# scienstanford/pbrt-v3-spectral

Measured on AMD Instinct MI355X. Metric: Mray/s (killeroo-simple, PathIntegrator maxdepth 5, Halton, SampledSpectrum-31, 1024 spp), higher is better.
Workload: dtype f32

## Files before the change

pbrt-v3-spectral_amd/csrc/device/pt_kernels.hip:

```cpp
#include <hip/hip_runtime.h>
#include <algorithm>
#include <chrono>
#include <cmath>
#include <cstdio>
#include <cstdlib>
#include <thread>
#include <cstring>
#include <string>
#include <vector>
#include <type_traits>
#include "d_sampling.h"
#include "d_texture.h"
#include "d_lens.h"

using namespace dpt;

#ifdef MIPT_PART
#define MIPT_HAS_MAIN (MIPT_PART == 0)
#else
#define MIPT_HAS_MAIN 1
#endif

namespace dptk {

// ... 8 lines not shown
        if (e_ != hipSuccess) {                                                           \
            g_err = std::string(#x) + ": " + hipGetErrorString(e_);                       \
            return MI_ERR_HIP;                                                            \
        }                                                                                 \
    } while (0)

constexpr int BLOCK = 256;
#ifndef MIPT_STACK_LDS
#define MIPT_STACK_LDS 12
#endif
constexpr int STACK_LDS = MIPT_STACK_LDS;
constexpr int STACK_SPILL = 64 - STACK_LDS;
static_assert(STACK_LDS >= 1 && STACK_LDS <= 63 && STACK_LDS * BLOCK * 12 <= 160 * 1024, "MIPT_STACK_LDS: 1..63 entries, and the block's stack must fit the CU's LDS");

enum : int {
    P_FILMX = 0, P_FILMY,
    P_TENC0, P_TENC1, P_TENC2, P_TENC3,
    P_COUNT
};
constexpr int P_WEIGHT = P_COUNT;
constexpr int P_LENSDIFF = P_COUNT + 1, N_LENSDIFF = 12;
enum : int {
    R_RAY0 = 0,
    R_RAY1,
    R_SH0, R_SH1,
    R_MI0, R_MI1,
    R_HIT,
    R_COUNT
};
constexpr int NQ = 8;
enum : int {
    Q_L = 0,
    Q_BETA = NQ,
    Q_LB = 2 * NQ,
    Q_LMIS = 3 * NQ,
    Q_COUNT = 4 * NQ,
    Q_LCA = Q_COUNT
};
DEV float Get4(const float4 &v, int k) { return k == 0 ? v.x : (k == 1 ? v.y : (k == 2 ? v.z : v.w)); }
DEV void Set4(float4 &v, int k, float x) { if (k == 0) v.x = x; else if (k == 1) v.y = x; else if (k == 2) v.z = x; else v.w = x; }
enum : int { I_HITPRIM = 0, I_PIXEL, I_SAMPLE, I_IDXLO, I_IDXHI, I_DIM , I_FLAGS, I_MISLIGHT,
             I_NPEND, I_PEND0, I_PEND1, I_PEND2, I_PEND3,
             I_BAND,
             I_HITINST,
             I_COUNT };
constexpr int MAX_PEND = 4;
constexpr int PEND_OVERFLOW = 0x100;
enum : int {
    F_ALIVE = 1, F_FINISHED = 2, F_SPECULAR = 4, F_SHADOW = 8, F_MIS = 16, F_NEE = 32, F_A_ADDED = 64,
    F_L_IN_B = 128,
    F_L_ZERO = 256,
    F_BETA_ONE = 512,
    F_DIFF = 1024,
    F_CAND = 2048, F_NEE_NZ = 4096,
    F_MIS_DARK = 8192
};
constexpr int FLAG_BITS = 14, FLAG_MASK = (1 << FLAG_BITS) - 1, BOUNCE_SHIFT = 14, DIM_SHIFT = 22;
static_assert(F_MIS_DARK < (1 << FLAG_BITS), "slot flags outgrew their field");
DEV int LPlane(int flags) { return (flags & F_L_IN_B) ? Q_LB : Q_L; }
DEV int LOtherPlane(int flags) { return (flags & F_L_IN_B) ? Q_L : Q_LB; }
DEV int StateWord(int flags, int bounces, int dim) { return (flags & FLAG_MASK) | ((bounces & 0xff) << BOUNCE_SHIFT) | (int)((unsigned)(dim & 0x3ff) << DIM_SHIFT); }
DEV int StateBounces(int word) { return (word >> BOUNCE_SHIFT) & 0xff; }
DEV int StateDim(int word) { return (int)((unsigned)word >> DIM_SHIFT); }
DEV bool RaySpanInBox(const V3 &o, const V3 &d, const float4 &bmin, const float4 &bmax, float *spanLo, float *spanHi) {
    float t0 = 0.f, t1 = kInfinity;
    const float oo[3] = {o.x, o.y, o.z}, dd[3] = {d.x, d.y, d.z}, lo[3] = {bmin.x, bmin.y, bmin.z}, hi[3] = {bmax.x, bmax.y, bmax.z};
#pragma unroll
    for (int a = 0; a < 3; ++a) {
        if (dd[a] == 0.f) { if (oo[a] < lo[a] || oo[a] > hi[a]) return false; continue; }
        const float inv = 1.f / dd[a];
        float ta = (lo[a] - oo[a]) * inv, tb = (hi[a] - oo[a]) * inv;
        if (ta > tb) { const float tt = ta; ta = tb; tb = tt; }
        tb *= 1.0001f;
        if (ta > t0) t0 = ta;
        if (tb < t1) t1 = tb;
    }
    *spanLo = t0; *spanHi = t1;
    return !(t0 > t1);
}
constexpr unsigned MIS_EXCL_BITS = 27, MIS_EXCL_NONE = (1u << MIS_EXCL_BITS) - 1u;
DEV void MisSpanWords(float lo, float hi, unsigned prim, float *tHi, float *word) {
    const float w = 1.f - lo / hi;
    int c = 126 - (int)((__float_as_uint(w) >> 23) & 0xffu);
    if (!(w > 0.f)) c = 20;
    c = (lo > 0.f && hi < kInfinity) ? max(0, min(c, 20)) : 0;
    *tHi = hi;
    *word = __uint_as_float(prim | ((unsigned)c << MIS_EXCL_BITS));
}

constexpr int MAX_CLASSES = 16;
constexpr int MISS_CLASS = 15;

struct Pool {
    float *f;
    float4 *q;
    float4 *r;
    int *i;
    uint32_t *shadowQ, *misQ;
    uint32_t *extQ;
    uint32_t *shadeQ;
    uint32_t *ovfQ;
    uint32_t n;
    __host__ __device__ __forceinline__ size_t ScalarIndex(int plane, uint32_t slot) const { return (size_t)plane * n + slot; }
    __host__ __device__ __forceinline__ size_t QuadIndex(int plane, uint32_t slot) const { return (((size_t)(plane >> 3) * n + slot) << 3) + (plane & 7); }
    __host__ __device__ __forceinline__ size_t RecordIndex(int plane, uint32_t slot) const {
        return plane < R_HIT ? (((size_t)(plane >> 1) * n + slot) << 1) + (plane & 1) : (size_t)plane * n + slot;
    }
    DEV float &F(int plane, uint32_t slot) const { return f[ScalarIndex(plane, slot)]; }
    DEV float4 &Q(int plane, uint32_t slot) const { return q[QuadIndex(plane, slot)]; }
    DEV float4 &R(int plane, uint32_t slot) const { return plane < R_HIT ? r[RecordIndex(plane, slot)] : r[ScalarIndex(plane, slot)]; }
    DEV int &I(int plane, uint32_t slot) const { return i[ScalarIndex(plane, slot)]; }
};

constexpr int STAT_STRIPES = 64;
struct alignas(128) DevStats {
    unsigned long long cameraRays, regularRays, shadowRays, totalPaths, zeroRadiancePaths, pathLengthSum, nodesVisited,
        triTests, badSamples, extendNodes, extendTris, extendRays;
};
struct alignas(128) DevCursor {
    unsigned int v;
};
struct DevCounters {
    DevStats stats[STAT_STRIPES];
    alignas(128) unsigned long long nextWork;
    DevCursor alive;
    DevCursor shadowCount, misCount;
    DevCursor primCount, contCount;
    DevCursor shadeCount[MAX_CLASSES];
    DevCursor travNext[3];
    DevCursor ovfCount[3];
};
constexpr size_t ITER_CLEAR_BYTES = sizeof(DevCursor) * (5 + MAX_CLASSES + 3 + 3);
DEV DevStats &Stats(DevCounters *ctr) { return ctr->stats[blockIdx.x & (STAT_STRIPES - 1)]; }
// ... 387 lines not shown
    (void)excl; (void)tLo; (void)ambiguous;
    const unsigned travChunk = (total >= (1u << 23)) ? 2u * (unsigned)TRAV_CHUNK : (unsigned)TRAV_CHUNK;
    const float4 *__restrict__ primTri = s.primTri;
    unsigned nodeCount = 0, triCount = 0, rayCount = 0;
    bool has = false;
    uint32_t slot = 0;
    unsigned myEntry = 0;
    RayCtx r;
    InitRayCtx(r, 0, 0, 0, 1, 1, 1);
    float tMax = 0;
    TravState st;
    st.cur = -1; st.sp = 0;
    TravSpill spill;
    int nPend = 0, hitPrim = -1;
    float hitT = 0, hitB0 = 0, hitB1 = 0, hitB2 = 0;
    int leafOff = 0, leafCnt = 0;
    bool leafSimple = false;
    __shared__ int sTask[BLOCK];
    int curInst = -1, hitInst = -1;
    bool hitInCur = false;
    TriRay triRay;
    triRay.kz = 2; triRay.Sx = triRay.Sy = 0; triRay.Sz = 1;
    bool exhausted = false;
#ifdef MIPT_TRAV_STATS
    unsigned long long dbgPasses = 0, dbgHas = 0, dbgWalk = 0, dbgWalkPasses = 0, dbgTriPasses = 0, dbgTri = 0;
#endif
    unsigned chunkNext = 0, chunkEnd = 0;
    while (true) {
        if (!exhausted) {
            const unsigned long long idle = __ballot(!has);
            if (idle) {
                if (chunkNext == chunkEnd) {
                    unsigned base = 0;
                    if (wlane == 0) base = atomicAdd(&ctr->travNext[QM].v, travChunk);
                    base = __shfl(base, 0, 64);
                    chunkNext = min(base, total);
                    chunkEnd = min(base + travChunk, total);
                    if (base >= total) exhausted = true;
                }
                const unsigned first = chunkNext;
                chunkNext = min(chunkNext + (unsigned)__popcll(idle), chunkEnd);
                if (!has) {
                    const unsigned my = first + __popcll(idle & ((1ull << wlane) - 1));
                    if (my < chunkEnd) {
                        if (MODE == 0) slot = queue[(my < nPrim) ? my : pool.n - nCont + (my - nPrim)];
                        else slot = queue[my];
                        if (MODE != 0) myEntry = my;
                        {
                            const float4 r0 = pool.R((MODE == 0) ? R_RAY0 : ((MODE == 1) ? R_SH0 : R_MI0), slot);
                            const float4 r1 = pool.R((MODE == 0) ? R_RAY1 : ((MODE == 1) ? R_SH1 : R_MI1), slot);
                            if (MODE == 0) InitRayCtx(r, r0.x, r0.y, r0.z, r1.x, r1.y, r1.z);
                            else InitRayCtx(r, r0.x, r0.y, r0.z, r0.w, r1.x, r1.y);
                            tMax = (MODE == 0) ? r0.w : ((MODE == 1) ? 1 - kShadowEpsilon : (MISANY ? r1.z : kInfinity));
                            if (MISANY) {
                                const unsigned xw = __float_as_uint(r1.w);
                                excl = (int)(xw & MIS_EXCL_NONE);
                                const unsigned code = xw >> MIS_EXCL_BITS;
                                tLo = code == 0 ? 0.f : tMax * (1.f - __uint_as_float((127u - code) << 23));
                                ambiguous = false;
                            }
                            StartTraversal(s, r, tMax, st, nodeCount);
                            triRay = MakeTriRay(V3(r.dx, r.dy, r.dz));
                            nPend = 0; hitPrim = -1;
                            hitT = hitB0 = hitB1 = hitB2 = 0;
                            leafCnt = 0;
                            curInst = hitInst = -1; hitInCur = false;
                            ++rayCount;
                            if (st.cur >= 0) has = true;
                            else if (MODE == 1) pool.shadowQ[pool.n + myEntry] = 0u;
                            else if (MODE == 2) {
                                *reinterpret_cast<uint2 *>(pool.misQ + pool.n + 2 * (size_t)myEntry) = make_uint2(0xffffffffu, 0u);
                                pool.R(R_HIT, slot) = make_float4(0.f, 0.f, 0.f, 0.f);
                            } else if (MISANY) {
                                *reinterpret_cast<uint2 *>(pool.misQ + pool.n + 2 * (size_t)myEntry) = make_uint2(0xffffffffu, 0u);
                            } else {
                                pool.I(I_HITPRIM, slot) = -1;
                                pool.I(I_NPEND, slot) = 0;
                                if (INST && MODE == 0) pool.I(I_HITINST, slot) = -1;
                                if (!ANY) pool.R(R_HIT, slot) = make_float4(0.f, 0.f, 0.f, 0.f);
                            }
                        }
                    }
                }
            }
        }
        if (!__any(has)) {
            if (exhausted) break;
            continue;
        }
        while (true) {
            const bool walking = has && st.cur >= 0;
            const bool inLeaf = has && leafCnt > 0;
            const int nLeaf = __popcll(__ballot(inLeaf));
            const bool anyWalk = __any(walking);
#ifdef MIPT_TRAV_STATS
            ++dbgPasses; dbgHas += __popcll(__ballot(has)); dbgWalk += __popcll(__ballot(walking));
            if (anyWalk) ++dbgWalkPasses;
            if (nLeaf > 0 && (nLeaf >= TRI_BATCH || !anyWalk)) { ++dbgTriPasses; dbgTri += nLeaf; }
#endif
            bool needPop = false, got = false, finished = false;
            int tkChild = 0, tkMeta = 0;
            if (walking) {
                if (__any(r.slow)) got = OpenNode<W, !ANY, false>(s.wnodes, st.cur, r, tMax, spill, lane, st.sp, &tkChild, &tkMeta, nodeCount);
                else got = OpenNode<W, !ANY, W == 4>(s.wnodes, st.cur, r, tMax, spill, lane, st.sp, &tkChild, &tkMeta, nodeCount);
                needPop = !got;
                st.cur = -1;
            }
            const bool triPass = nLeaf > 0 && (nLeaf >= TRI_BATCH || !anyWalk);
            if (triPass && __any(inLeaf && leafSimple)) {
                const bool coop = inLeaf && leafSimple;
                const int want = coop ? min(leafCnt, COOP_KMAX) : 0;
                int base = 0, total = 0;
#pragma unroll
                for (int b = 0; b < COOP_KMAX; ++b) {
                    const unsigned long long m = __ballot(want > b);
                    base += __popcll(m & ((1ull << wlane) - 1));
                    total += __popcll(m);
                }
                const int grant = max(0, min(want, 64 - base));
                int *taskOwner = &sTask[threadIdx.x & ~63];
                for (int k = 0; k < grant; ++k) taskOwner[base + k] = wlane | (k << 8);
                __builtin_amdgcn_fence(__ATOMIC_RELEASE, "wavefront");
                __builtin_amdgcn_wave_barrier();
                const int nTask = min(total, 64);
                const bool worker = wlane < nTask;
                const int ow = worker ? taskOwner[wlane] : wlane;
                const int owner = ow & 63, tk = ow >> 8;
// ... 48 lines not shown
                            const int src = rem ? base + k : wlane;
                            const float dk = __shfl(rDet, src, 64), tsk = __shfl(rTs, src, 64), tk2 = __shfl(rT, src, 64);
                            if (rem) {
                                const bool beyond = dk < 0 ? (tsk < cur * dk) : (tsk > cur * dk);
                                if (!beyond) { cur = tk2; win = k; }
                                rem &= rem - 1u;
                            }
                        }
                    }
                    if (!multi && seg) win = __ffs(seg) - 1;
                    const int src = win >= 0 ? base + win : wlane;
                    const float hT = __shfl(rT, src, 64), hB0 = __shfl(rB0, src, 64), hB1 = __shfl(rB1, src, 64), hB2 = __shfl(rB2, src, 64);
                    if (win >= 0) {
                        tMax = hT;
                        hitPrim = leafOff + win; hitT = hT; hitB0 = hB0; hitB1 = hB1; hitB2 = hB2;
                        if (INST) { hitInst = curInst; hitInCur = true; }
                    }
                    triCount += (unsigned)grant;
                }
                if (grant > 0) {
                    leafOff += grant; leafCnt -= grant;
                    needPop = !finished && leafCnt == 0;
                }
            }
            if (triPass && inLeaf && !leafSimple) {
                const int prim = leafOff;
                ++leafOff; --leafCnt;
                const float4 v0 = primTri[3 * prim];
                const unsigned pf = __float_as_uint(v0.w);
                bool entered = false;
                if (INST && (pf & PRIM_FLAG_INSTANCE)) {
                    const int k = __float_as_int(primTri[3 * prim + 1].w);
                    StackPush<!ANY>(spill, lane, st.sp, leafOff, -(leafCnt + 1), tMax);
                    const Ray ir = XfRay(s.instances[k].w2i, Ray(V3(r.ox, r.oy, r.oz), V3(r.dx, r.dy, r.dz), tMax));
                    InitRayCtx(r, ir.o.x, ir.o.y, ir.o.z, ir.d.x, ir.d.y, ir.d.z);
                    triRay = MakeTriRay(ir.d);
                    tMax = ir.tMax;
                    curInst = k; hitInCur = false;
                    leafCnt = 0;
                    const float4 bMin = s.instRootBounds[2 * k], bMax = s.instRootBounds[2 * k + 1];
                    float tBox;
                    ++nodeCount;
                    got = BoxTest(r, bMin.x, bMin.y, bMin.z, bMax.x, bMax.y, bMax.z, tMax, &tBox);
                    tkChild = s.instWideRoot[k]; tkMeta = 0;
                    entered = true;
                } else if (INST && curInst >= 0 && (pf & PRIM_FLAG_SPHERE)) {
                    float t;
                    if (SphereHitT(s.spheres[__float_as_int(primTri[3 * prim + 1].w)], V3(r.ox, r.oy, r.oz), V3(r.dx, r.dy, r.dz), tMax, &t)) {
                        if (ANY) { hitPrim = prim; finished = true; }
                        else { tMax = t; hitPrim = prim; hitT = t; hitB0 = hitB1 = hitB2 = 0; hitInst = curInst; hitInCur = true; }
                    }
                } else
                if (MISANY && prim == excl) {}
                else if (pf & PRIM_FLAG_SPHERE) {
                    if ((nPend & 0xff) < MAX_PEND) {
                        pool.I(I_PEND0 + (nPend & 0xff), slot) = prim;
                        if (!ANY) pool.F(P_TENC0 + (nPend & 0xff), slot) = tMax;
                        ++nPend;
                    }
                    else nPend |= PEND_OVERFLOW;
                } else {
                    const float4 v1 = primTri[3 * prim + 1], v2 = primTri[3 * prim + 2];
                    ++triCount;
                    TriHit th;
                    if (TriTestRay(V3(v0.x, v0.y, v0.z), V3(v1.x, v1.y, v1.z), V3(v2.x, v2.y, v2.z), V3(r.ox, r.oy, r.oz),
                                   triRay, tMax, &th)) {
                        bool counts = true;
                        if constexpr (ALPHA)
                            if (pf & PRIM_FLAG_ALPHA)
                                counts = !(pf & PRIM_FLAG_DEGENERATE) && AlphaPass(s, __float_as_int(v1.w), th.b0, th.b1, th.b2, PSEM);
                        if (!counts) {}
                        else if (PSEM) { hitPrim = prim; finished = true; }
                        else if (MISANY) {
                            if (!(pf & PRIM_FLAG_DEGENERATE)) {
                                if (th.t < tLo) { hitPrim = prim; finished = true; }
                                else ambiguous = true;
                            }
                        }
                        else if (!(pf & PRIM_FLAG_DEGENERATE)) {
                            tMax = th.t;
                            hitPrim = prim; hitT = th.t; hitB0 = th.b0; hitB1 = th.b1; hitB2 = th.b2;
                            if (INST) { hitInst = curInst; hitInCur = true; }
                        }
                    }
                }
                needPop = entered ? !got : (!finished && leafCnt == 0);
            }
            if (needPop) {
                while (!got && st.sp > 0) {
                    float t;
                    StackPop<!ANY>(spill, lane, st.sp, &tkChild, &tkMeta, &t);
                    if (INST && tkMeta < 0) {
                        const float4 r0 = pool.R((MODE == 0) ? R_RAY0 : ((MODE == 1) ? R_SH0 : R_MI0), slot);
                        const float4 r1 = pool.R((MODE == 0) ? R_RAY1 : ((MODE == 1) ? R_SH1 : R_MI1), slot);
                        if (MODE == 0) InitRayCtx(r, r0.x, r0.y, r0.z, r1.x, r1.y, r1.z);
                        else InitRayCtx(r, r0.x, r0.y, r0.z, r0.w, r1.x, r1.y);
                        triRay = MakeTriRay(V3(r.dx, r.dy, r.dz));
                        if (!hitInCur) tMax = ANY ? 1 - kShadowEpsilon : t;
                        curInst = -1;
                        tkMeta = -tkMeta - 1;
                        got = tkMeta > 0;
                        continue;
                    }
                    got = ANY || t < tMax;
                }
                finished = !got;
            }
            if (got) {
                if (tkMeta > 0) { leafOff = tkChild; leafCnt = tkMeta & LEAF_COUNT_MASK; leafSimple = (tkMeta & LEAF_SIMPLE) != 0; }
                else st.cur = tkChild;
            }
            if (finished && MODE == 1) {
                pool.shadowQ[pool.n + myEntry] = (hitPrim >= 0 ? 0x80000000u : 0u) | (unsigned)nPend;
                has = false;
                leafCnt = 0;
            } else
            if (finished && MODE == 2) {
                *reinterpret_cast<uint2 *>(pool.misQ + pool.n + 2 * (size_t)myEntry) = make_uint2((unsigned)hitPrim, (unsigned)nPend);
                pool.R(R_HIT, slot) = make_float4(hitT, hitB0, hitB1, hitB2);
                has = false;
                leafCnt = 0;
            } else
            if (finished && MISANY) {
                *reinterpret_cast<uint2 *>(pool.misQ + pool.n + 2 * (size_t)myEntry) = make_uint2(hitPrim >= 0 ? (unsigned)hitPrim : (ambiguous ? 0xfffffffeu : 0xffffffffu), (unsigned)nPend);
                has = false;
                leafCnt = 0;
            } else
            if (finished) {
                pool.I(I_HITPRIM, slot) = hitPrim;
                pool.I(I_NPEND, slot) = nPend;
                if (!ANY) pool.R(R_HIT, slot) = make_float4(hitT, hitB0, hitB1, hitB2);
                if (INST && MODE == 0) pool.I(I_HITINST, slot) = hitInst;
                has = false;
                leafCnt = 0;
            }
            const int active = __popcll(__ballot(has));
            if (active == 0 || (!exhausted && active < REFILL_BELOW)) break;
        }
    }
#ifdef MIPT_TRAV_STATS
    if (blockIdx.x == 7 && threadIdx.x == 0 && total > 1000000)
        printf("TRAVSTAT mode %d total %u passes %llu has/pass %.1f walkPasses %llu walk/walkPass %.1f triPasses %llu tri/triPass %.1f\n", MODE, total, dbgPasses,
               (double)dbgHas / dbgPasses, dbgWalkPasses, (double)dbgWalk / (dbgWalkPasses ? dbgWalkPasses : 1), dbgTriPasses, (double)dbgTri / (dbgTriPasses ? dbgTriPasses : 1));
#endif
    DevStats &st8 = Stats(ctr);
    if (MODE == 1) CountAdd(&st8.shadowRays, rayCount);
    else CountAdd(&st8.regularRays, rayCount);
    CountAdd(&st8.nodesVisited, nodeCount);
    CountAdd(&st8.triTests, triCount);
    if (MODE == 0) { CountAdd(&st8.extendNodes, nodeCount); CountAdd(&st8.extendTris, triCount); CountAdd(&st8.extendRays, rayCount); }
}

template <bool ANY>
DEV bool ResolveQuadrics(const DScene &s, const Pool &pool, uint32_t slot, const V3 &ro, const V3 &rd, float tMaxIn, Hit *h, bool foundTri, int np) {
    if (ANY) {
        for (int j = 0; j < (np & 0xff); ++j) {
            const int prim = pool.I(I_PEND0 + j, slot);
            float t;
            if (SphereHitT(s.spheres[__float_as_int(s.primTri[3 * prim + 1].w)], ro, rd, tMaxIn, &t)) return true;
        }
        return foundTri;
    }
    float tBest = kInfinity, tEncBest = 0.f;
    int primBest = -1;
    for (int j = 0; j < (np & 0xff); ++j) {
        const int prim = pool.I(I_PEND0 + j, slot);
        const float tEnc = pool.F(P_TENC0 + j, slot);
        float t;
        if (SphereHitT(s.spheres[__float_as_int(s.primTri[3 * prim + 1].w)], ro, rd, minf(tEnc, tBest), &t)) { tBest = t; primBest = prim; tEncBest = tEnc; }
    }
    if (primBest < 0) return foundTri;
    if (foundTri && tEncBest > h->t && h->t <= tBest) return true;
    h->prim = primBest; h->t = tBest; h->b0 = h->b1 = h->b2 = 0; h->inst = -1;
    return true;
}
template <bool ANY, bool INST>
DEV bool Retraverse(const DScene &s, const V3 &ro, const V3 &rd, float tMax, Hit *h) {
// ... 113 lines not shown
        const unsigned rank = ((ch < 4 ? rankLo >> (8 * ch) : rankHi >> (8 * (ch - 4))) & 255u);
        const uint32_t slot = (blockIdx.x * SLOT_CHUNKS + ch) * BLOCK + threadIdx.x;
        pool.shadeQ[(size_t)cls * pool.n + sBase[cls] + sCnt[ch][wave][cls] + rank] = slot;
    }
    CountAdd(&Stats(ctr).pathLengthSum, pathLen);
}

DEV int CommitShadowVerdict(int flags, bool occluded, unsigned &zero) {
    const bool added = !occluded && (flags & F_NEE_NZ);
    if (!occluded) flags = (flags ^ F_L_IN_B) & ~F_L_ZERO;
    flags &= ~(F_SHADOW | F_CAND | F_NEE_NZ);
    if (flags & F_MIS) { if (added) flags |= F_A_ADDED; }
    else { if (!added) ++zero; flags &= ~(F_NEE | F_A_ADDED); }
    return flags;
}

template <bool INST>
__global__ void __launch_bounds__(BLOCK) k_resolve_shadow(DScene s, Pool pool, DevCounters *ctr) {
    const unsigned count = ctr->shadowCount.v;
    unsigned zero = 0;
    for (uint32_t qi = blockIdx.x * BLOCK + threadIdx.x; qi < count; qi += gridDim.x * BLOCK) {
        const uint32_t slot = pool.shadowQ[qi];
        const int flags = pool.I(I_FLAGS, slot);
        const unsigned verdict = pool.shadowQ[pool.n + qi];
        bool occluded = (verdict >> 31) != 0u;
        const int npend = occluded ? 0 : (int)(verdict & 0x7fffffffu);
        if (npend & PEND_OVERFLOW) { pool.ovfQ[(size_t)pool.n + atomicAdd(&ctr->ovfCount[1].v, 1u)] = slot; continue; }
        if (npend != 0) {
            const float4 r0 = pool.R(R_SH0, slot), r1 = pool.R(R_SH1, slot);
            Hit h;
            occluded = ResolveQuadrics<true>(s, pool, slot, PackedRayO(r0), PackedRayD(r0, r1), 1 - kShadowEpsilon, &h, false, npend);
        }
        pool.I(I_FLAGS, slot) = CommitShadowVerdict(flags, occluded, zero);
    }
    CountAdd(&Stats(ctr).zeroRadiancePaths, zero);
}

DEV bool AddMisContribution(const Pool &pool, uint32_t slot, int &flags) {
    bool added = false;
    const bool lZero = (flags & F_L_ZERO) != 0;
    for (int c = 0; c < NQ; ++c) {
        const float4 a = pool.Q(Q_LMIS + c, slot);
        added |= (a.x != 0.f) | (a.y != 0.f) | (a.z != 0.f) | (a.w != 0.f);
        float4 l = make_float4(0.f, 0.f, 0.f, 0.f);
        if (!lZero) l = pool.Q(LPlane(flags) + c, slot);
        l.x += a.x; l.y += a.y; l.z += a.z; l.w += a.w;
        pool.Q(LPlane(flags) + c, slot) = l;
    }
    flags &= ~F_L_ZERO;
    return added;
}
DEV void CloseMisEstimate(const Pool &pool, uint32_t slot, int flags, bool added, unsigned &zero) {
    if (!added && !(flags & F_A_ADDED)) ++zero;
    pool.I(I_FLAGS, slot) = flags & ~(F_NEE | F_MIS | F_A_ADDED | F_MIS_DARK);
}

DEV void LoadMisRay(const Pool &pool, uint32_t slot, V3 &ro, V3 &rd, Hit &h, bool &have) {
    if (have) return;
    const float4 r0 = pool.R(R_MI0, slot), r1 = pool.R(R_MI1, slot), hr = pool.R(R_HIT, slot);
    ro = PackedRayO(r0); rd = PackedRayD(r0, r1);
    if (h.prim >= 0) SetHitRecord(&h, hr);
    have = true;
}
template <bool INST, bool OVF>
DEV bool MisClosestHit(const DScene &s, const Pool &pool, uint32_t slot, int npend, V3 &ro, V3 &rd, Hit &h, bool &haveRay) {
    bool found = h.prim >= 0;
    if (npend != 0) {
        LoadMisRay(pool, slot, ro, rd, h, haveRay);
        if constexpr (OVF) found = Retraverse<false, INST>(s, ro, rd, kInfinity, &h);
        else found = ResolveQuadrics<false>(s, pool, slot, ro, rd, kInfinity, &h, found, npend);
    }
    return found;
}

template <bool INST, bool OVF>
DEV void ResolveMisSlot(const DScene &s, const Pool &pool, DevCounters *ctr, uint32_t slot, int hitPrim, int npend, unsigned &zero) {
    int flags = pool.I(I_FLAGS, slot);
    V3 ro, rd;
    Hit h;
    h.prim = hitPrim; h.t = 0.f; h.b0 = h.b1 = h.b2 = 0.f;
    bool haveRay = false;
    if (!OVF && (npend & PEND_OVERFLOW)) { pool.ovfQ[2 * (size_t)pool.n + atomicAdd(&ctr->ovfCount[2].v, 1u)] = slot; return; }
    const bool found = MisClosestHit<INST, OVF>(s, pool, slot, npend, ro, rd, h, haveRay);
    bool added = false;
    const int misLight = s.nLights > 1 ? pool.I(I_MISLIGHT, slot) : 0;
    if (!found && s.lights[misLight].type == MI_LIGHT_INFINITE) added |= AddMisContribution(pool, slot, flags);
    if (found) {
        const int lightNum = misLight;
        if (s.prims[h.prim].area_light == lightNum && !(flags & F_MIS_DARK)) {
            const mi_light &l = s.lights[lightNum];
            bool emit = l.two_sided != 0;
            if (!emit) {
                LoadMisRay(pool, slot, ro, rd, h, haveRay);
                SurfaceInteraction li;
                HitInteraction(s, h.prim, ro, rd, h.b0, h.b1, h.b2, &li);
                emit = Dot(li.n, -rd) > 0;
            }
            if (emit) added |= AddMisContribution(pool, slot, flags);
        }
    }
    CloseMisEstimate(pool, slot, flags, added, zero);
}
DEV void ResolveMisVisibility(const DScene &s, const Pool &pool, DevCounters *ctr, uint32_t slot, int word0, int npend, unsigned &zero) {
    int flags = pool.I(I_FLAGS, slot);
    const bool dark = (flags & F_MIS_DARK) != 0;
    bool exact = !dark && (npend & PEND_OVERFLOW) != 0, add = false;
    if (!exact && !dark) {
        const int misLight = s.nLights > 1 ? pool.I(I_MISLIGHT, slot) : 0;
        const mi_light &l = s.lights[misLight];
        if (l.type == MI_LIGHT_INFINITE) {
            bool found = word0 >= 0;
            if (!found && (npend & 0xff)) {
                const float4 r0 = pool.R(R_MI0, slot), r1 = pool.R(R_MI1, slot);
                Hit h;
                found = ResolveQuadrics<true>(s, pool, slot, PackedRayO(r0), PackedRayD(r0, r1), kInfinity, &h, false, npend);
            }
            add = !found;
        } else if (word0 >= 0) {}
        else if (word0 == -2 || (npend & 0xff)) exact = true;
        else {
            const float4 r0 = pool.R(R_MI0, slot), r1 = pool.R(R_MI1, slot);
            const V3 ro = PackedRayO(r0), rd = PackedRayD(r0, r1);
            if (l.shape < 0) {
                const mi_sphere &sp = s.spheres[~l.shape];
                SurfaceInteraction li;
                float t, t2;
                if (SphereInteraction(sp, ro, rd, kInfinity, &li, &t)) {
                    if (!SphereHitT(sp, ro, rd, r1.z, &t2)) exact = true;
                    else add = l.two_sided != 0 || Dot(li.n, -rd) > 0;
                }
            } else if (l.two_sided != 0) add = true;
            else {
                const int32_t *v = &s.triIndices[3 * l.shape];
                TriHit th;
                if (TriTest(LoadV3(s.P, v[0]), LoadV3(s.P, v[1]), LoadV3(s.P, v[2]), ro, rd, kInfinity, &th)) {
                    SurfaceInteraction li;
                    TriInteraction(s, l.shape, th.b0, th.b1, th.b2, rd, &li);
                    add = Dot(li.n, -rd) > 0;
                }
            }
        }
    }
    if (exact) { pool.ovfQ[2 * (size_t)pool.n + atomicAdd(&ctr->ovfCount[2].v, 1u)] = slot; return; }
    const bool added = add && AddMisContribution(pool, slot, flags);
    CloseMisEstimate(pool, slot, flags, added, zero);
}
template <bool INST>
__global__ void __launch_bounds__(BLOCK) k_resolve_mis(DScene s, Pool pool, DevCounters *ctr) {
    const unsigned count = ctr->misCount.v;
    unsigned zero = 0;
    for (uint32_t qi = blockIdx.x * BLOCK + threadIdx.x; qi < count; qi += gridDim.x * BLOCK) {
        const uint2 v = *reinterpret_cast<const uint2 *>(pool.misQ + pool.n + 2 * (size_t)qi);
        if (!INST && s.misAny) ResolveMisVisibility(s, pool, ctr, pool.misQ[qi], (int)v.x, (int)v.y, zero);
        else ResolveMisSlot<INST, false>(s, pool, ctr, pool.misQ[qi], (int)v.x, (int)v.y, zero);
    }
    CountAdd(&Stats(ctr).zeroRadiancePaths, zero);
}

constexpr int OVERFLOW_GRID = 512;
template <bool INST>
__global__ void __launch_bounds__(BLOCK) k_resolve_overflow(DScene s, Pool pool, DevCounters *ctr, int mode) {
    const unsigned count = ctr->ovfCount[mode].v;
    unsigned zero = 0, pathLen = 0;
    for (unsigned qi = blockIdx.x * BLOCK + threadIdx.x; qi < count; qi += gridDim.x * BLOCK) {
        const uint32_t slot = pool.ovfQ[(size_t)mode * pool.n + qi];
        if (mode == 0) {
            const float4 r0 = pool.R(R_RAY0, slot), r1 = pool.R(R_RAY1, slot);
            Hit h;
            h.prim = -1; h.t = 0.f; h.b0 = h.b1 = h.b2 = 0.f;
            const bool found = Retraverse<false, INST>(s, V3(r0.x, r0.y, r0.z), V3(r1.x, r1.y, r1.z), r0.w, &h);
            const int prim = found ? h.prim : -1;
            pool.I(I_HITPRIM, slot) = prim;
            pool.R(R_HIT, slot) = HitRecord(h);
            if (INST) pool.I(I_HITINST, slot) = h.inst;
            const int word = pool.I(I_FLAGS, slot);
            if (EndsUnshaded(word, prim, s.maxDepth, s.nInfiniteLights)) { pool.I(I_FLAGS, slot) = FinishedWord(word); pathLen += (unsigned)StateBounces(word); }
            else {
                const int cls = ClassOfPrim(s.primTri, prim);
                pool.shadeQ[(size_t)cls * pool.n + atomicAdd(&ctr->shadeCount[cls].v, 1u)] = slot;
            }
        } else if (mode == 1) {
            const float4 r0 = pool.R(R_SH0, slot), r1 = pool.R(R_SH1, slot);
            Hit h;
            const bool occluded = Retraverse<true, INST>(s, PackedRayO(r0), PackedRayD(r0, r1), 1 - kShadowEpsilon, &h);
            pool.I(I_FLAGS, slot) = CommitShadowVerdict(pool.I(I_FLAGS, slot), occluded, zero);
        } else
            ResolveMisSlot<INST, true>(s, pool, ctr, slot, -1, PEND_OVERFLOW, zero);
    }
    CountAdd(&Stats(ctr).zeroRadiancePaths, zero);
    CountAdd(&Stats(ctr).pathLengthSum, pathLen);
}

template <bool MOVING = false>
DEV void CameraRay(const DScene &s, float pFilmX, float pFilmY, float lensU, float lensV, Ray *out, float timeU = 0.f, float *timeOut = nullptr) {
    const mi_camera &cam = s.camera;
    V3 pCamera = XfPoint(cam.raster_to_camera, V3(pFilmX, pFilmY, 0));
    V3 dir = Normalize(V3(pCamera.x, pCamera.y, pCamera.z));
    Ray ray(V3(0, 0, 0), dir);
    if (cam.lens_radius > 0) {
        float dx, dy;
        ConcentricSampleDisk(lensU, lensV, &dx, &dy);
        float lx = cam.lens_radius * dx, ly = cam.lens_radius * dy;
        float ft = cam.focal_distance / ray.d.z;
        V3 pFocus = ray.at(ft);
        ray.o = V3(lx, ly, 0);
// ... 398 lines not shown
    ts->dpdv = XfVector(m, ts->dpdv);
    ts->shDpdv = XfVector(m, ts->shDpdv);
    ts->dndu = XfNormal(mInv, ts->dndu);
    ts->dndv = XfNormal(mInv, ts->dndv);
}

DEV void HitInteraction(const DScene &s, int prim, const V3 &ro, const V3 &rd, float b0, float b1, float b2, SurfaceInteraction *si) {
    const mi_prim p = s.prims[prim];
    if (p.shape >= 0) TriInteraction(s, p.shape, b0, b1, b2, rd, si);
    else { float t; SphereInteraction(s.spheres[~p.shape], ro, rd, kInfinity, si, &t); }
}


DEV float4 LoadBeta(const Pool &pool, int c, uint32_t slot, bool betaOne) {
    float4 bt = make_float4(1.f, 1.f, 1.f, 1.f);
    if (!betaOne) bt = pool.Q(Q_BETA + c, slot);
    return bt;
}

struct SpectrumTile {
    float4 q[NQ][BLOCK];
    int slotOf[BLOCK];
    unsigned char laneOf[BLOCK], specOf[BLOCK];
};
DEV void StoreSpectrumLines(SpectrumTile &t, const Pool &pool, int spectrum, uint32_t slot, bool wrote) {
    const int lane = threadIdx.x & 63, wbase = threadIdx.x & ~63;
    const unsigned long long lt = (1ull << lane) - 1ull;
    const unsigned long long active = __ballot(1), wmask = __ballot(wrote);
    const int nW = __popcll(wmask), nGroups = __popcll(active) >> 3;
    if (nGroups == 0) {
        if (wrote) for (int c = 0; c < NQ; ++c) pool.Q(spectrum + c, slot) = t.q[c][threadIdx.x];
        return;
    }
    if (wrote) {
        const int rw = __popcll(wmask & lt);
        t.slotOf[wbase + rw] = (int)slot;
        t.laneOf[wbase + rw] = (unsigned char)lane;
        t.specOf[wbase + rw] = (unsigned char)spectrum;
    }
    __builtin_amdgcn_fence(__ATOMIC_RELEASE, "wavefront");
    __builtin_amdgcn_wave_barrier();
    const int ra = __popcll(active & lt), g = ra >> 3, c = ra & 7;
    if (g < nGroups)
        for (int e = g; e < nW; e += nGroups)
            pool.Q((int)t.specOf[wbase + e] + c, (uint32_t)t.slotOf[wbase + e]) = t.q[c][wbase + t.laneOf[wbase + e]];
    __builtin_amdgcn_fence(__ATOMIC_ACQUIRE, "wavefront");
    __builtin_amdgcn_wave_barrier();
}

#ifndef MIPT_SHADE_WAVES_PER_EU
#define MIPT_SHADE_WAVES_PER_EU 4
#endif

template <int NL, unsigned TM, bool LENS = false>
__global__ void __launch_bounds__(BLOCK) __attribute__((amdgpu_waves_per_eu(MIPT_SHADE_WAVES_PER_EU, 8))) k_shade(DScene s, Pool pool, DevCounters *ctr, unsigned classes) {
    unsigned blk = blockIdx.x, count = 0;
    int cls = -1;
    for (int c = 0; c < MAX_CLASSES; ++c) {
        if (!((classes >> c) & 1)) continue;
        const unsigned n = ctr->shadeCount[c].v, nb = (n + BLOCK - 1) / BLOCK;
        if (blk < nb) { cls = c; count = n; break; }
        blk -= nb;
    }
    const uint32_t qi = blk * BLOCK + threadIdx.x;
    constexpr bool HALTON_ONLY = (TM & TM_SAMPLERS) == 0;
    constexpr bool SIMPLE_SPECTRA = NL <= 2 && TM_SIMPLE_KINDS(TM);
    constexpr bool ACCUM = NL > 2 || (TM & TM_TEXTURED) != 0;
    __shared__ SpectrumTile tile;
    auto rdTile = [&](int c) -> float4 { return tile.q[c][threadIdx.x]; };
    auto wrTile = [&](int c, const float4 &v) { tile.q[c][threadIdx.x] = v; };
    unsigned totalPaths = 0, pathLen = 0, zeroNow = 0;
    bool wantShadow = false, wantMis = false;
    uint32_t slot = 0;
    if (cls >= 0 && qi < count) {
        slot = pool.shadeQ[(size_t)cls * pool.n + qi];
        const int word = pool.I(I_FLAGS, slot);
        const int flags = word & FLAG_MASK;
        bool lZero = (flags & F_L_ZERO) != 0, betaWritten = false;
        const int lPlane = LPlane(flags);
        const bool betaOne = (flags & F_BETA_ONE) != 0;
        const int bounces = StateBounces(word);
        int dimNow = StateDim(word);
        const int prim = pool.I(I_HITPRIM, slot);
        const bool found = prim >= 0;
        auto loadBeta = [&](int c) -> float4 { return LoadBeta(pool, c, slot, betaOne); };
        const bool emitCheck = bounces == 0 || (flags & F_SPECULAR);
        const bool needIsect = found && (bounces < s.maxDepth || emitCheck);
        const bool needRay = needIsect || (!found && emitCheck && TM_LIGHT(TM, MI_LIGHT_INFINITE) && s.nInfiniteLights > 0);
        float4 ray0 = make_float4(0.f, 0.f, 0.f, 0.f), ray1 = make_float4(0.f, 0.f, 1.f, 1.f);
        if (needRay) { ray0 = pool.R(R_RAY0, slot); ray1 = pool.R(R_RAY1, slot); }
        V3 ro(ray0.x, ray0.y, ray0.z), rd(ray1.x, ray1.y, ray1.z);
        SurfaceInteraction isect;
        bool finished = false, passThrough = false;
        int inst = -1;
        V3 roS = ro, rdS = rd;
        if constexpr ((TM & TM_INSTANCES) != 0) {
            if (needIsect) inst = pool.I(I_HITINST, slot);
            if (inst >= 0) { const Ray ir = XfRay(s.instances[inst].w2i, Ray(ro, rd, kInfinity)); roS = ir.o; rdS = ir.d; }
        }
        if (needIsect) { const float4 hr = pool.R(R_HIT, slot); HitInteraction(s, prim, roS, rdS, hr.y, hr.z, hr.w, &isect); }
        SurfaceInteraction isectObj;
        if constexpr ((TM & TM_INSTANCES) != 0) {
            if (inst >= 0) { isectObj = isect; InteractionToWorld(s.instances[inst], &isect); }
        }
        if ((bounces == 0 || (flags & F_SPECULAR)) && found) {
            const int li = s.prims[prim].area_light;
// ... 390 lines not shown
                                            accF |= aF;
                                            return true;
                                        };
#pragma unroll 1
                                        for (int c = 0; c < NQ; ++c)
                                            if (!quad(c, std::false_type{})) quad(c, std::true_type{});
                                    }
                                    if (go && !dark) {
                                        auto quad = [&](int c, auto exactTag) {
                                            constexpr bool EXACT = decltype(exactTag)::value;
                                            DivTrack trk;
                                            trk.Reset(divFast);
                                            const float4 bt = loadBeta(c);
                                            float4 fq = SimpleEvalQuad<NL, TM, EXACT>(sl, bx, c, trk), Lq = isEnvLight ? zero4 : LoadSpec4(light.L, c);
                                            if (c == NQ - 1) { fq.w = 0.f; Lq.w = 0.f; }
                                            unsigned aF = 0u;
                                            float o[4];
#pragma unroll
                                            for (int k = 0; k < 4; ++k) {
                                                const float f = Get4(fq, k) * absdot;
                                                OrNonZero(aF, f);
                                                const float LiB = isEnvLight ? ((4 * c + k < MI_NSPEC) ? IllumBin(s, envLe, min(4 * c + k, MI_NSPEC - 1)) : 0.f) : Get4(Lq, k);
                                                const float x = (f * LiB) * weight;
                                                float Ld;
                                                if constexpr (EXACT) { Ld = DivBy(x, spDiv); if (!selIsOne) Ld = DivBy(Ld, selDiv); }
                                                else {
                                                    Ld = DivFast(x, spDiv.d, spDiv.r, trk);
                                                    if (!allSelOne) { const float Ld2 = DivFast(Ld, selDiv.d, selDiv.r, trk); Ld = selIsOne ? Ld : Ld2; }
                                                }
                                                o[k] = Get4(bt, k) * Ld;
                                            }
                                            if (!EXACT && __any(trk.Bad())) return false;
                                            tile.q[c][threadIdx.x] = make_float4(o[0], o[1], o[2], o[3]);
                                            accF |= aF;
                                            return true;
                                        };
#pragma unroll 1
                                        for (int c = 0; c < NQ; ++c)
                                            if (!quad(c, std::false_type{})) quad(c, std::true_type{});
                                    }
                                    fNonBlack |= accF != 0u;
                                } else {
                                    if (dark) {
#pragma unroll 1
                                        for (int c = 0; c < NQ; ++c) darkQuad(c, fQuad(c));
                                    }
                                    if (go && !dark) {
#pragma unroll 1
                                        for (int c = 0; c < NQ; ++c) misQuad(c, fQuad(c), isEnvLight ? zero4 : LoadSpec4(light.L, c));
                                    }
                                }
                                StoreSpectrumLines(tile, pool, Q_LMIS, slot, go && !dark);
                                if (fNonBlack && go) {
                                    if (dark) newFlags |= F_MIS_DARK;
                                    pool.R(R_MI0, slot) = make_float4(mr.o.x, mr.o.y, mr.o.z, mr.d.x);
                                    pool.R(R_MI1, slot) = make_float4(mr.d.y, mr.d.z, misTHi, misWord);
                                    if (s.nLights > 1) pool.I(I_MISLIGHT, slot) = lightNum;
                                    newFlags |= F_MIS;
                                }
                            }
                        }
                    }
                }
            }
            {
                V3 wo = -rd, wi;
                float pdf = 0;
                int sflags = 0;
                float u2[2];
                Get2D<HALTON_ONLY>(s, ps, pixelPlane, samplePlane, slot, &u2[0], &u2[1]);
                const float u0 = u2[0], u1 = u2[1];
                BSDFEvalT<NL> ev;
                V3 wiLocal;
                const bool ok = BSDF_Sample_f<NL, TM, !ACCUM>(fr, wo, &wi, u0, u1, &pdf, MI_BSDF_ALL, &sflags, &ev, &wiLocal);
                if constexpr (ACCUM) {
                    if (ok && pdf != 0.f) {
                        if (ev.n > 0) AccumulateSpecular<NL, TM>(ev.lobes[0], mat->bxdf, ltp, rdTile, wrTile);
                        else AccumulateFLocal<NL, TM>(fr, fr.WorldToLocal(wo), wiLocal, Dot(wi, fr.ng) * Dot(wo, fr.ng) > 0, MI_BSDF_ALL, ltp, rdTile, wrTile);
                    }
                }
                auto fQuad = [&](int c) -> float4 { if constexpr (ACCUM) return rdTile(c); else return EvalQuad<NL, TM>(ev, mat->bxdf, c, ltp); };
                bool fNonBlack = false;
                if (ok && pdf != 0.f) {
                    const float absdot = AbsDot(wi, isect.shN);
                    float etaScale = ray1.w;
                    if ((sflags & MI_BSDF_SPECULAR) && (sflags & MI_BSDF_TRANSMISSION)) {
                        float eta = mat->eta;
                        etaScale *= (Dot(wo, isect.n) > 0) ? (eta * eta) : 1 / (eta * eta);
                    }
                    const Divisor pdfDiv = MakeDivisor(pdf);
                    float maxRR = 0;
                    auto contQuad = [&](int c, const float4 &fq) {
                        float4 bt = loadBeta(c);
#pragma unroll
                        for (int k = 0; k < 4; ++k) {
                            const int b = 4 * c + k;
                            if (b < MI_NSPEC) {
                                const float f = Get4(fq, k);
                                fNonBlack |= (f != 0.f);
                                const float nb = Get4(bt, k) * DivBy(f * absdot, pdfDiv);
                                Set4(bt, k, nb);
                                const float rr = nb * etaScale;
                                maxRR = (b == 0) ? rr : maxf(maxRR, rr);
                            }
                        }
                        tile.q[c][threadIdx.x] = bt;
                    };
                    if constexpr (SIMPLE_SPECTRA) {
                        const SimpleLobes<NL> sl = MakeSimpleLobes<NL, TM>(ev);
                        const mi_bxdf *bx = mat->bxdf;
                        const bool divFast = sl.divisorsFast && pdfDiv.fast;
// ... 26 lines not shown
                            return true;
                        };
#pragma unroll 1
                        for (int c = 0; c < NQ; ++c)
                            if (!quad(c, std::false_type{})) quad(c, std::true_type{});
                        fNonBlack |= accF != 0u;
                    } else {
#pragma unroll 1
                        for (int c = 0; c < NQ; ++c) contQuad(c, fQuad(c));
                    }
                    bool killed = false;
                    if (fNonBlack) {
                        if (maxRR < s.rrThreshold && bounces > 3) {
                            float q = maxf(.05f, 1 - maxRR);
                            if (Get1D<HALTON_ONLY>(s, ps, pixelPlane, samplePlane, slot) < q) killed = true;
                            else {
                                const Divisor inv = MakeDivisor(1 - q);
#pragma unroll 1
                                for (int c = 0; c < NQ; ++c) {
                                    float4 bt = tile.q[c][threadIdx.x];
#pragma unroll
                                    for (int k = 0; k < 4; ++k)
                                        if (4 * c + k < MI_NSPEC) Set4(bt, k, DivBy(Get4(bt, k), inv));
                                    tile.q[c][threadIdx.x] = bt;
                                }
                            }
                        }
                    }
                    const bool needBeta = fNonBlack && !killed && (bounces + 1 < s.maxDepth || (sflags & MI_BSDF_SPECULAR));
                    StoreSpectrumLines(tile, pool, Q_BETA, slot, needBeta);
                    if (needBeta) betaWritten = true;
                    if (fNonBlack) {
                        if (killed) finished = true;
                        else {
                            const Ray nr = SpawnRay(isect, wi);
                            pool.R(R_RAY0, slot) = make_float4(nr.o.x, nr.o.y, nr.o.z, nr.tMax);
                            pool.R(R_RAY1, slot) = make_float4(nr.d.x, nr.d.y, nr.d.z, etaScale);
                            if (sflags & MI_BSDF_SPECULAR) newFlags |= F_SPECULAR;
                        }
                    }
                }
                if (!(ok && pdf != 0.f && fNonBlack)) finished = true;
            }
            dimNow = ps.dim;
            if constexpr (!HALTON_ONLY) { if (IsPixelSampler(s)) { pool.I(I_DIM, slot) = ps.dim; dimNow = 0; } }
            if (!HALTON_ONLY && s.samplerType >= MI_SAMPLER_RANDOM) {
                pool.I(I_IDXLO, slot) = (int)(uint32_t)ps.index;
                pool.I(I_IDXHI, slot) = (int)(uint32_t)(ps.index >> 32);
            }
        }
        if (!passThrough) {
            if (finished) {
                pathLen = (unsigned)bounces;
                newFlags = (newFlags & (F_NEE | F_SHADOW | F_MIS | F_CAND | F_NEE_NZ | F_MIS_DARK)) | F_FINISHED;
            } else {
                newFlags |= F_ALIVE;
            }
            if (lZero) newFlags |= F_L_ZERO;
            newFlags |= flags & F_L_IN_B;
            if (betaOne && !betaWritten) newFlags |= F_BETA_ONE;
            wantShadow = (newFlags & F_SHADOW) != 0;
            wantMis = (newFlags & F_MIS) != 0;
            if ((newFlags & F_NEE) && !wantShadow && !wantMis) { ++zeroNow; newFlags &= ~F_NEE; }
            pool.I(I_FLAGS, slot) = StateWord(newFlags, finished ? bounces : bounces + 1, dimNow);
        }
    }
    __shared__ unsigned sAppend[10];
    unsigned posS, posM;
    BlockReserve2(&ctr->shadowCount.v, wantShadow, &ctr->misCount.v, wantMis, sAppend, &posS, &posM);
    if (wantShadow) pool.shadowQ[posS] = slot;
    if (wantMis) pool.misQ[posM] = slot;
    {
        unsigned packed = totalPaths | (zeroNow << 8) | (pathLen << 16);
        for (int off = 32; off > 0; off >>= 1) packed += __shfl_down(packed, off, 64);
        if ((threadIdx.x & 63) == 0 && packed) {
            DevStats &st8 = Stats(ctr);
            if (packed & 0xffu) atomicAdd(&st8.totalPaths, (unsigned long long)(packed & 0xffu));
            if ((packed >> 8) & 0xffu) atomicAdd(&st8.zeroRadiancePaths, (unsigned long long)((packed >> 8) & 0xffu));
            if (packed >> 16) atomicAdd(&st8.pathLengthSum, (unsigned long long)(packed >> 16));
        }
    }
}

#if MIPT_HAS_MAIN
__global__ void k_build_spatial(DScene s, float *func, float *cdf, float *funcInt, uint32_t nVox) {
    const uint32_t vox = blockIdx.x * blockDim.x + threadIdx.x;
    if (vox >= nVox) return;
    const int nL = (int)s.nLights;
    int pi[3];
    pi[0] = vox % s.nVoxels[0];
    pi[1] = (vox / s.nVoxels[0]) % s.nVoxels[1];
    pi[2] = vox / (s.nVoxels[0] * s.nVoxels[1]);
    float lo[3], hi[3];
    for (int i = 0; i < 3; ++i) {
        float t0 = (float)pi[i] / (float)s.nVoxels[i], t1 = (float)(pi[i] + 1) / (float)s.nVoxels[i];
        float a = lerpf(t0, s.wbMin[i], s.wbMax[i]), b = lerpf(t1, s.wbMin[i], s.wbMax[i]);
        lo[i] = minf(a, b); hi[i] = maxf(a, b);
    }
    float *f = func + (size_t)vox * nL;
    for (int j = 0; j < nL; ++j) f[j] = 0.f;
    const int nSamples = 128;
    for (int i = 0; i < nSamples; ++i) {
        float t[3] = {RadicalInverse(s, 0, i), RadicalInverse(s, 1, i), RadicalInverse(s, 2, i)};
        Interaction intr;
        intr.p = V3(lerpf(t[0], lo[0], hi[0]), lerpf(t[1], lo[1], hi[1]), lerpf(t[2], lo[2], hi[2]));
        intr.wo = V3(1, 0, 0);
        float u0 = RadicalInverse(s, 3, i), u1 = RadicalInverse(s, 4, i);
        for (int j = 0; j < nL; ++j) {
            const mi_light &l = s.lights[j];
            LightSample ls = SampleLi<TM_ALL>(s, l, intr, u0, u1);
            if (ls.pdf > 0) {
                float yy = 0.f;
                if (!ls.black) for (int b = 0; b < MI_NSPEC; ++b) yy += s.cieY[b] * LiBin<TM_ALL>(s, l, ls, b);
                f[j] += YScale(yy) / ls.pdf;
            }
        }
// ... 953 lines not shown
            const mi_mesh &m = d->meshes[d->tri_mesh[p.shape]];
            if (DegenerateTriangle(d, v, m, a, b, c)) flags |= PRIM_FLAG_DEGENERATE;
            if (m.alpha_tex >= 0 || m.shadow_alpha_tex >= 0) { flags |= PRIM_FLAG_ALPHA; hasAlphaMasks = true; }
        } else {
            hasQuadrics = true;
            flags |= PRIM_FLAG_SPHERE;
            shapeIdx = ~p.shape;
        }
        flags |= (unsigned)(p.material >= 0 ? matClass[p.material] : MISS_CLASS) << PRIM_CLASS_SHIFT;
        memcpy(&a.w, &flags, 4);
        memcpy(&b.w, &shapeIdx, 4);
        pt3[3 * i] = a; pt3[3 * i + 1] = b; pt3[3 * i + 2] = c;
    }
    return pt3;
}

std::vector<float4> BuildLightBounds(const mi_scene_desc *d) {
    std::vector<float4> lb((size_t)std::max<uint32_t>(d->n_lights, 1) * 2, float4{-INFINITY, -INFINITY, -INFINITY, 0});
    for (uint32_t i = 0; i < d->n_lights; ++i) {
        const mi_light &l = d->lights[i];
        float mn[3] = {INFINITY, INFINITY, INFINITY}, mx[3] = {-INFINITY, -INFINITY, -INFINITY};
        auto add = [&](float x, float y, float z) { const float p[3] = {x, y, z}; for (int a = 0; a < 3; ++a) { mn[a] = std::min(mn[a], p[a]); mx[a] = std::max(mx[a], p[a]); } };
        bool have = false;
        if (l.type == MI_LIGHT_DIFFUSE_AREA && l.shape >= 0 && (uint32_t)l.shape < d->n_tris) {
            const int32_t *v = &d->tri_indices[3 * l.shape];
            for (int k = 0; k < 3; ++k) add(d->P[3 * v[k]], d->P[3 * v[k] + 1], d->P[3 * v[k] + 2]);
            have = true;
        } else if (l.type == MI_LIGHT_DIFFUSE_AREA && l.shape < 0 && (uint32_t)(~l.shape) < d->n_spheres) {
            const mi_sphere &sp = d->spheres[~l.shape];
            for (int c = 0; c < 8; ++c) {
                const float x = (c & 1) ? sp.radius : -sp.radius, y = (c & 2) ? sp.radius : -sp.radius, z = (c & 4) ? sp.z_max : sp.z_min;
                const float *m = sp.o2w;
                const float w = m[12] * x + m[13] * y + m[14] * z + m[15];
                add((m[0] * x + m[1] * y + m[2] * z + m[3]) / w, (m[4] * x + m[5] * y + m[6] * z + m[7]) / w, (m[8] * x + m[9] * y + m[10] * z + m[11]) / w);
            }
            have = true;
        }
        if (have) {
            float scale = 0;
            for (int a = 0; a < 3; ++a) scale = std::max(scale, std::max(std::abs(mn[a]), std::abs(mx[a])) + (mx[a] - mn[a]));
            const float e = 1e-3f * scale;
            lb[2 * i] = float4{mn[0] - e, mn[1] - e, mn[2] - e, 0};
            lb[2 * i + 1] = float4{mx[0] + e, mx[1] + e, mx[2] + e, 0};
        } else {
            lb[2 * i] = float4{-INFINITY, -INFINITY, -INFINITY, 0};
            lb[2 * i + 1] = float4{INFINITY, INFINITY, INFINITY, 0};
        }
    }
    return lb;
}

std::vector<int> BuildLightPrims(const mi_scene_desc *d, bool &misAny) {
    std::vector<int> lp((size_t)std::max<uint32_t>(d->n_lights, 1), (int)MIS_EXCL_NONE), seen((size_t)std::max<uint32_t>(d->n_lights, 1), 0);
    bool ok = d->n_instances == 0 && d->n_prims < MIS_EXCL_NONE;
    for (uint32_t i = 0; i < d->n_prims; ++i) {
        const int al = d->prims[i].area_light;
        if (al < 0) continue;
        if ((uint32_t)al >= d->n_lights) { ok = false; continue; }
        lp[al] = (int)i;
        if (++seen[al] > 1 || d->prims[i].shape != d->lights[al].shape || d->prims[i].instance != 0) ok = false;
    }
    for (uint32_t i = 0; i < d->n_lights; ++i) {
        const mi_light &l = d->lights[i];
        if (l.type != MI_LIGHT_DIFFUSE_AREA) continue;
        if (!seen[i]) ok = false;
        if (l.shape >= 0 && (uint32_t)l.shape < d->n_tris) {
            const mi_mesh &m = d->meshes[d->tri_mesh[l.shape]];
            if (m.alpha_tex >= 0 || m.shadow_alpha_tex >= 0) ok = false;
        }
    }
#ifdef MIPT_NO_MIS_ANY
    ok = false;
#endif
    misAny = ok;
    return lp;
}

std::vector<uint64_t> BuildPrimeMagics(const mi_sampler &sm) {
    std::vector<uint64_t> magic(sm.n_dims);
    for (int i = 0; i < sm.n_dims; ++i) magic[i] = (~0ull) / (uint64_t)sm.primes[i] + 1;
    return magic;
}

std::vector<uint32_t> BuildPixelOffsets(const mi_sampler &sm) {
    std::vector<uint32_t> table(128 * 128, 0);
    if (sm.sample_stride <= 1) return table;
    auto inverseRadicalInverse = [](uint64_t base, uint64_t inverse, int nDigits) {
        uint64_t index = 0;
        for (int i = 0; i < nDigits; ++i) { uint64_t digit = inverse % base; inverse /= base; index = index * base + digit; }
        return index;
    };
    for (int py = 0; py < 128; ++py)
        for (int px = 0; px < 128; ++px) {
            int64_t offset = 0;
            const int pm[2] = {px, py};
            for (int i = 0; i < 2; ++i) {
                uint64_t dimOffset = inverseRadicalInverse(i == 0 ? 2 : 3, (uint64_t)pm[i], sm.base_exponents[i]);
                offset += (int64_t)(dimOffset * (uint64_t)(sm.sample_stride / sm.base_scales[i]) * (uint64_t)sm.mult_inverse[i]);
            }
            offset %= (int64_t)sm.sample_stride;
            table[py * 128 + px] = (uint32_t)offset;
        }
    return table;
}

std::vector<float> BuildEwaWeights() {
    std::vector<float> lut(128);
// ... 926 lines not shown
```

Baseline: 4826.

## Encode dark MIS rays in the ray exclusion word and skip their resolve

Replaces the per-slot F_MIS_DARK flag with a sentinel exclusion value carried in the MIS ray word. The traverse kernel writes a dark marker in the answer and skips R_HIT writes and sphere pending records for these rays, and the resolve kernel skips dark entries entirely. Dark rays are still traced for their RNG and visibility side effects but no longer touch I_MISLIGHT or the resolve path. This trims memory traffic and divergent work in the MIS resolve. The trade-off is one fewer usable primitive index and more coupling between the shade, traverse and resolve stages.

```diff
diff --git a/pbrt-v3-spectral_amd/csrc/device/pt_kernels.hip b/pbrt-v3-spectral_amd/csrc/device/pt_kernels.hip
--- a/pbrt-v3-spectral_amd/csrc/device/pt_kernels.hip
+++ b/pbrt-v3-spectral_amd/csrc/device/pt_kernels.hip
@@ -84,11 +84,10 @@
     F_L_ZERO = 256,
     F_BETA_ONE = 512,
     F_DIFF = 1024,
-    F_CAND = 2048, F_NEE_NZ = 4096,
-    F_MIS_DARK = 8192
+    F_CAND = 2048, F_NEE_NZ = 4096
 };
 constexpr int FLAG_BITS = 14, FLAG_MASK = (1 << FLAG_BITS) - 1, BOUNCE_SHIFT = 14, DIM_SHIFT = 22;
-static_assert(F_MIS_DARK < (1 << FLAG_BITS), "slot flags outgrew their field");
+static_assert(F_NEE_NZ < (1 << FLAG_BITS), "slot flags outgrew their field");
 DEV int LPlane(int flags) { return (flags & F_L_IN_B) ? Q_LB : Q_L; }
 DEV int LOtherPlane(int flags) { return (flags & F_L_IN_B) ? Q_L : Q_LB; }
 DEV int StateWord(int flags, int bounces, int dim) { return (flags & FLAG_MASK) | ((bounces & 0xff) << BOUNCE_SHIFT) | (int)((unsigned)(dim & 0x3ff) << DIM_SHIFT); }
@@ -111,6 +110,8 @@
     return !(t0 > t1);
 }
 constexpr unsigned MIS_EXCL_BITS = 27, MIS_EXCL_NONE = (1u << MIS_EXCL_BITS) - 1u;
+constexpr unsigned MIS_EXCL_DARK = MIS_EXCL_NONE - 1u;
+constexpr unsigned MIS_ANSWER_DARK = 0x80000000u;
 DEV void MisSpanWords(float lo, float hi, unsigned prim, float *tHi, float *word) {
     const float w = 1.f - lo / hi;
     int c = 126 - (int)((__float_as_uint(w) >> 23) & 0xffu);
@@ -604,6 +605,7 @@
                             if (MODE == 0) InitRayCtx(r, r0.x, r0.y, r0.z, r1.x, r1.y, r1.z);
                             else InitRayCtx(r, r0.x, r0.y, r0.z, r0.w, r1.x, r1.y);
                             tMax = (MODE == 0) ? r0.w : ((MODE == 1) ? 1 - kShadowEpsilon : (MISANY ? r1.z : kInfinity));
+                            if (MODE == 2) excl = (int)(__float_as_uint(r1.w) & MIS_EXCL_NONE);
                             if (MISANY) {
                                 const unsigned xw = __float_as_uint(r1.w);
                                 excl = (int)(xw & MIS_EXCL_NONE);
@@ -621,10 +623,11 @@
                             if (st.cur >= 0) has = true;
                             else if (MODE == 1) pool.shadowQ[pool.n + myEntry] = 0u;
                             else if (MODE == 2) {
-                                *reinterpret_cast<uint2 *>(pool.misQ + pool.n + 2 * (size_t)myEntry) = make_uint2(0xffffffffu, 0u);
-                                pool.R(R_HIT, slot) = make_float4(0.f, 0.f, 0.f, 0.f);
+                                const bool dark = excl == (int)MIS_EXCL_DARK;
+                                *reinterpret_cast<uint2 *>(pool.misQ + pool.n + 2 * (size_t)myEntry) = make_uint2(0xffffffffu, dark ? MIS_ANSWER_DARK : 0u);
+                                if (!dark) pool.R(R_HIT, slot) = make_float4(0.f, 0.f, 0.f, 0.f);
                             } else if (MISANY) {
-                                *reinterpret_cast<uint2 *>(pool.misQ + pool.n + 2 * (size_t)myEntry) = make_uint2(0xffffffffu, 0u);
+                                *reinterpret_cast<uint2 *>(pool.misQ + pool.n + 2 * (size_t)myEntry) = make_uint2(0xffffffffu, excl == (int)MIS_EXCL_DARK ? MIS_ANSWER_DARK : 0u);
                             } else {
                                 pool.I(I_HITPRIM, slot) = -1;
                                 pool.I(I_NPEND, slot) = 0;
@@ -779,6 +782,7 @@
                     }
                 } else
                 if (MISANY && prim == excl) {}
+                else if ((MODE >= 2) && (pf & PRIM_FLAG_SPHERE) && excl == (int)MIS_EXCL_DARK) {}
                 else if (pf & PRIM_FLAG_SPHERE) {
                     if ((nPend & 0xff) < MAX_PEND) {
                         pool.I(I_PEND0 + (nPend & 0xff), slot) = prim;
@@ -843,13 +847,14 @@
                 leafCnt = 0;
             } else
             if (finished && MODE == 2) {
-                *reinterpret_cast<uint2 *>(pool.misQ + pool.n + 2 * (size_t)myEntry) = make_uint2((unsigned)hitPrim, (unsigned)nPend);
-                pool.R(R_HIT, slot) = make_float4(hitT, hitB0, hitB1, hitB2);
+                const bool dark = excl == (int)MIS_EXCL_DARK;
+                *reinterpret_cast<uint2 *>(pool.misQ + pool.n + 2 * (size_t)myEntry) = make_uint2((unsigned)hitPrim, dark ? MIS_ANSWER_DARK : (unsigned)nPend);
+                if (!dark) pool.R(R_HIT, slot) = make_float4(hitT, hitB0, hitB1, hitB2);
                 has = false;
                 leafCnt = 0;
             } else
             if (finished && MISANY) {
-                *reinterpret_cast<uint2 *>(pool.misQ + pool.n + 2 * (size_t)myEntry) = make_uint2(hitPrim >= 0 ? (unsigned)hitPrim : (ambiguous ? 0xfffffffeu : 0xffffffffu), (unsigned)nPend);
+                *reinterpret_cast<uint2 *>(pool.misQ + pool.n + 2 * (size_t)myEntry) = make_uint2(hitPrim >= 0 ? (unsigned)hitPrim : (ambiguous ? 0xfffffffeu : 0xffffffffu), excl == (int)MIS_EXCL_DARK ? MIS_ANSWER_DARK : (unsigned)nPend);
                 has = false;
                 leafCnt = 0;
             } else
@@ -1069,7 +1074,7 @@
 }
 DEV void CloseMisEstimate(const Pool &pool, uint32_t slot, int flags, bool added, unsigned &zero) {
     if (!added && !(flags & F_A_ADDED)) ++zero;
-    pool.I(I_FLAGS, slot) = flags & ~(F_NEE | F_MIS | F_A_ADDED | F_MIS_DARK);
+    pool.I(I_FLAGS, slot) = flags & ~(F_NEE | F_MIS | F_A_ADDED);
 }
 
 DEV void LoadMisRay(const Pool &pool, uint32_t slot, V3 &ro, V3 &rd, Hit &h, bool &have) {
@@ -1104,7 +1109,7 @@
     if (!found && s.lights[misLight].type == MI_LIGHT_INFINITE) added |= AddMisContribution(pool, slot, flags);
     if (found) {
         const int lightNum = misLight;
-        if (s.prims[h.prim].area_light == lightNum && !(flags & F_MIS_DARK)) {
+        if (s.prims[h.prim].area_light == lightNum) {
             const mi_light &l = s.lights[lightNum];
             bool emit = l.two_sided != 0;
             if (!emit) {
@@ -1120,9 +1125,8 @@
 }
 DEV void ResolveMisVisibility(const DScene &s, const Pool &pool, DevCounters *ctr, uint32_t slot, int word0, int npend, unsigned &zero) {
     int flags = pool.I(I_FLAGS, slot);
-    const bool dark = (flags & F_MIS_DARK) != 0;
-    bool exact = !dark && (npend & PEND_OVERFLOW) != 0, add = false;
-    if (!exact && !dark) {
+    bool exact = (npend & PEND_OVERFLOW) != 0, add = false;
+    if (!exact) {
         const int misLight = s.nLights > 1 ? pool.I(I_MISLIGHT, slot) : 0;
         const mi_light &l = s.lights[misLight];
         if (l.type == MI_LIGHT_INFINITE) {
@@ -1168,6 +1172,7 @@
     unsigned zero = 0;
     for (uint32_t qi = blockIdx.x * BLOCK + threadIdx.x; qi < count; qi += gridDim.x * BLOCK) {
         const uint2 v = *reinterpret_cast<const uint2 *>(pool.misQ + pool.n + 2 * (size_t)qi);
+        if (v.y & MIS_ANSWER_DARK) continue;
         if (!INST && s.misAny) ResolveMisVisibility(s, pool, ctr, pool.misQ[qi], (int)v.x, (int)v.y, zero);
         else ResolveMisSlot<INST, false>(s, pool, ctr, pool.misQ[qi], (int)v.x, (int)v.y, zero);
     }
@@ -1672,6 +1677,7 @@
 #define MIPT_SHADE_WAVES_PER_EU 4
 #endif
 
+constexpr int SHADE_DARK_RAY = 1 << FLAG_BITS;
 template <int NL, unsigned TM, bool LENS = false>
 __global__ void __launch_bounds__(BLOCK) __attribute__((amdgpu_waves_per_eu(MIPT_SHADE_WAVES_PER_EU, 8))) k_shade(DScene s, Pool pool, DevCounters *ctr, unsigned classes) {
     unsigned blk = blockIdx.x, count = 0;
@@ -2168,11 +2174,11 @@
                                 }
                                 StoreSpectrumLines(tile, pool, Q_LMIS, slot, go && !dark);
                                 if (fNonBlack && go) {
-                                    if (dark) newFlags |= F_MIS_DARK;
+                                    if (dark) misWord = __uint_as_float(MIS_EXCL_DARK | (31u << MIS_EXCL_BITS));
                                     pool.R(R_MI0, slot) = make_float4(mr.o.x, mr.o.y, mr.o.z, mr.d.x);
                                     pool.R(R_MI1, slot) = make_float4(mr.d.y, mr.d.z, misTHi, misWord);
-                                    if (s.nLights > 1) pool.I(I_MISLIGHT, slot) = lightNum;
-                                    newFlags |= F_MIS;
+                                    if (s.nLights > 1 && !dark) pool.I(I_MISLIGHT, slot) = lightNum;
+                                    newFlags |= dark ? SHADE_DARK_RAY : F_MIS;
                                 }
                             }
                         }
@@ -2305,7 +2311,7 @@
         if (!passThrough) {
             if (finished) {
                 pathLen = (unsigned)bounces;
-                newFlags = (newFlags & (F_NEE | F_SHADOW | F_MIS | F_CAND | F_NEE_NZ | F_MIS_DARK)) | F_FINISHED;
+                newFlags = (newFlags & (F_NEE | F_SHADOW | F_MIS | F_CAND | F_NEE_NZ | SHADE_DARK_RAY)) | F_FINISHED;
             } else {
                 newFlags |= F_ALIVE;
             }
@@ -2313,8 +2319,8 @@
             newFlags |= flags & F_L_IN_B;
             if (betaOne && !betaWritten) newFlags |= F_BETA_ONE;
             wantShadow = (newFlags & F_SHADOW) != 0;
-            wantMis = (newFlags & F_MIS) != 0;
-            if ((newFlags & F_NEE) && !wantShadow && !wantMis) { ++zeroNow; newFlags &= ~F_NEE; }
+            wantMis = (newFlags & (F_MIS | SHADE_DARK_RAY)) != 0;
+            if ((newFlags & F_NEE) && !wantShadow && !(newFlags & F_MIS)) { ++zeroNow; newFlags &= ~F_NEE; }
             pool.I(I_FLAGS, slot) = StateWord(newFlags, finished ? bounces : bounces + 1, dimNow);
         }
     }
@@ -3374,7 +3380,7 @@
 
 std::vector<int> BuildLightPrims(const mi_scene_desc *d, bool &misAny) {
     std::vector<int> lp((size_t)std::max<uint32_t>(d->n_lights, 1), (int)MIS_EXCL_NONE), seen((size_t)std::max<uint32_t>(d->n_lights, 1), 0);
-    bool ok = d->n_instances == 0 && d->n_prims < MIS_EXCL_NONE;
+    bool ok = d->n_instances == 0 && d->n_prims < MIS_EXCL_DARK;
     for (uint32_t i = 0; i < d->n_prims; ++i) {
         const int al = d->prims[i].area_light;
         if (al < 0) continue;
```

Measured after the change: 4882, median of 6. 1.01x the previous value.
